# jinli99/iShapEditing

Measured on AMD Instinct MI355X. Metric: end-to-end drag-edit wall-clock (s) per shape, lower is better.
Workload: dtype f16; 1 GPU; C3 chair drag-edit: 3 handle->target pairs, 40 guided iterations (UNet fwd + drag gradient + UNet input-grad bwd + DDPM update) + 256^3 occupancy decode; unet=421M params, 1x96x128x128 latent, fp16 torso, r1=12, scale=1200

## Files before the change

include/ishap.h:

```cpp
#ifndef ISHAP_H
#define ISHAP_H
#ifdef __cplusplus
extern "C" {
#endif

const char* ishap_last_error(void);
int ishap_device_status(void);
int ishap_rendezvous_would_grant(const void* owner, void* stream);
int ishap_version(void);

typedef struct ishap_unet ishap_unet;

typedef struct {
  int image_size;
  int in_channels;
  int model_channels;
  int out_channels;
  int num_res_blocks;
  int n_mult;
  int channel_mult[8];
  int n_att;
  int attention_ds[8];
  int num_head_channels;
  int max_batch;
// ... 96 lines not shown
                        const float* grad_mul_dev, long long numel, float* out, void* stream);
int ishap_axpby(const float* x, const float* y, float a, float b, long long numel, float* out, void* stream);

typedef struct {
  int W;
  int ld;
  int Cc;
  const int* chmap;
  const float* sources;
  const float* targets;
  int B;
  int r;
  float voxel;
  float cof;
  int l1;
  unsigned char* touched;
  int* nmask;
  void* acc;
  void* grad_fx;
  unsigned char* chan_weight;
  const float* weights;
} ishap_drag_args;
int ishap_drag_setup(const ishap_drag_args* a, void* stream);
int ishap_drag_loss_grad(const ishap_drag_args* a, const void* edit_nhwc_f16, const void* orig_nhwc_f16,
                         float* grad_nhwc, float* loss, void* stream);
int ishap_drag_loss_cotangent(const ishap_drag_args* a, const void* edit_nhwc_f16, const void* orig_nhwc_f16,
                              float* grad_nhwc, float* loss, void* cot_f16, unsigned* bits, float* scale2, void* stream);
typedef struct {
  int E;
  int W, ld, Cc;
  const int* chmap;
  const float* sources;
  const float* targets;
  const int* handle_offsets;
  int r;
  float voxel;
  const float* cof;
  int l1;
  long long orig_stride;
  void* scratch;
  long long scratch_bytes;
  const float* weights;
  long long weights_stride;
} ishap_drag_batch_args;
long long ishap_drag_batch_scratch_bytes(int E, int W, int ld);
int ishap_drag_batch_setup(const ishap_drag_batch_args* a, void* stream);
// ... 244 lines not shown
```

ishapediting_amd/_lib.py:

```python
from __future__ import annotations

import ctypes as C
import os

HERE = os.path.dirname(os.path.abspath(__file__))
LIB_PATH = os.path.join(HERE, "libishap_hip.so")

c_float_p = C.POINTER(C.c_float)
c_void_p = C.c_void_p


class UNetConfigC(C.Structure):
    _fields_ = [("image_size", C.c_int), ("in_channels", C.c_int), ("model_channels", C.c_int),
                ("out_channels", C.c_int), ("num_res_blocks", C.c_int), ("n_mult", C.c_int),
                ("channel_mult", C.c_int * 8), ("n_att", C.c_int), ("attention_ds", C.c_int * 8),
                ("num_head_channels", C.c_int), ("max_batch", C.c_int)]


class StepCoefs(C.Structure):
    _fields_ = [("min_log", C.c_float), ("max_log", C.c_float), ("sqrt_recip", C.c_float),
                ("sqrt_recipm1", C.c_float), ("coef1", C.c_float), ("coef2", C.c_float),
                ("nonzero", C.c_float), ("clip_denoised", C.c_int), ("mode", C.c_int),
                ("ddim_a", C.c_float), ("ddim_b", C.c_float), ("ddim_sigma", C.c_float),
                ("rng", C.c_int), ("rng_seed", C.c_ulonglong), ("rng_offset", C.c_ulonglong), ("noise_out", c_void_p)]
# ... 92 lines not shown
    "ishap_unet_run_tail": (C.c_int, [c_void_p]),
    "ishap_unet_snapshot_save": (C.c_int, [c_void_p, c_void_p]),
    "ishap_unet_snapshot_restore": (C.c_int, [c_void_p, c_void_p]),
    "ishap_unet_snapshot_drop": (C.c_int, [c_void_p]),
    "ishap_unet_snapshot_bytes": (C.c_longlong, [c_void_p]),
    "ishap_unet_marks": (C.c_int, [c_void_p, c_void_p, c_void_p, C.c_int, c_void_p, c_void_p]),
    "ishap_unet_prepare_timesteps": (C.c_int, [c_void_p, c_void_p, C.c_int, c_void_p]),
    "ishap_unet_backward_input": (C.c_int, [c_void_p, c_void_p, c_void_p, c_void_p, c_void_p]),
    "ishap_unet_backward_from_output": (C.c_int, [c_void_p, c_void_p, C.c_int, c_void_p, c_void_p, c_void_p]),
    "ishap_triplane_points_loss_grad": (C.c_int, [c_void_p, C.c_int, C.POINTER(DecoderWeightsC), c_void_p, c_void_p, c_void_p,
                                                  c_void_p, C.c_longlong, c_void_p, c_void_p, c_void_p, c_void_p]),
    "ishap_x0_grad_to_cotangent": (C.c_int, [c_void_p, c_void_p, c_void_p, c_void_p, C.c_float, C.c_float, C.c_int, C.c_int,
                                             c_void_p, c_void_p, c_void_p]),
    "ishap_ddpm_step": (C.c_int, [c_void_p, c_void_p, c_void_p, c_void_p, C.POINTER(StepCoefs), C.c_int, C.c_int,
                                  C.c_int, c_void_p, c_void_p, c_void_p, c_void_p, c_void_p]),
    "ishap_ddpm_step_guided": (C.c_int, [c_void_p, c_void_p, c_void_p, c_void_p, C.POINTER(StepCoefs), C.c_int, C.c_int, C.c_int,
                                         c_void_p, C.c_float, c_void_p, c_void_p, c_void_p, c_void_p, c_void_p]),
    "ishap_ddpm_step_guided_scales": (C.c_int, [c_void_p, c_void_p, c_void_p, c_void_p, C.POINTER(StepCoefs), C.c_int, C.c_int,
                                                C.c_int, c_void_p, c_void_p, c_void_p, c_void_p, c_void_p, c_void_p, c_void_p]),
    "ishap_guided_update": (C.c_int, [c_void_p, c_void_p, c_void_p, C.c_float, c_void_p, C.c_longlong, c_void_p,
                                      c_void_p]),
    "ishap_axpby": (C.c_int, [c_void_p, c_void_p, C.c_float, C.c_float, C.c_longlong, c_void_p, c_void_p]),
    "ishap_drag_setup": (C.c_int, [C.POINTER(DragArgsC), c_void_p]),
    "ishap_drag_loss_grad": (C.c_int, [C.POINTER(DragArgsC), c_void_p, c_void_p, c_void_p, c_void_p, c_void_p]),
    "ishap_drag_loss_cotangent": (C.c_int, [C.POINTER(DragArgsC), c_void_p, c_void_p, c_void_p, c_void_p, c_void_p, c_void_p,
                                            c_void_p, c_void_p]),
    "ishap_drag_batch_scratch_bytes": (C.c_longlong, [C.c_int, C.c_int, C.c_int]),
    "ishap_drag_batch_setup": (C.c_int, [C.POINTER(DragBatchArgsC), c_void_p]),
    "ishap_drag_batch_loss_grad": (C.c_int, [C.POINTER(DragBatchArgsC), c_void_p, c_void_p, c_void_p, c_void_p, c_void_p]),
    "ishap_drag_batch_loss_cotangent": (C.c_int, [C.POINTER(DragBatchArgsC), c_void_p, c_void_p, c_void_p, c_void_p, c_void_p,
                                                  c_void_p, c_void_p, c_void_p]),
    "ishap_drag_track_scratch_bytes": (C.c_longlong, [C.c_int] * 5),
    "ishap_drag_track": (C.c_int, [c_void_p, c_void_p, C.c_longlong, C.c_int, C.c_int, C.c_int, c_void_p, c_void_p,
                                   C.POINTER(C.c_int), C.c_int, C.c_float, C.c_int, C.c_int, c_void_p, c_void_p, c_void_p, c_void_p,
                                   c_void_p, c_void_p, C.c_longlong, c_void_p]),
    "ishap_drag_retarget": (C.c_int, [C.POINTER(DragArgsC), c_void_p, c_void_p, C.c_float, C.c_float, c_void_p, c_void_p, c_void_p,
                                      c_void_p]),
    "ishap_drag_batch_retarget": (C.c_int, [C.POINTER(DragBatchArgsC), c_void_p, c_void_p, C.c_float, C.c_float, c_void_p, c_void_p,
                                            c_void_p, c_void_p]),
    "ishap_drag_batch_retarget_each": (C.c_int, [C.POINTER(DragBatchArgsC), c_void_p, c_void_p, C.POINTER(C.c_float),
                                                 C.POINTER(C.c_float), c_void_p, c_void_p, c_void_p, c_void_p]),
    "ishap_region_plane_weights_scratch_bytes": (C.c_longlong, [C.c_int]),
    "ishap_region_plane_weights": (C.c_int, [c_void_p, C.c_int, c_void_p, c_void_p, C.c_int, C.c_int, C.c_int, C.c_float, C.c_float,
                                             c_void_p, c_void_p, c_void_p, C.c_longlong, c_void_p]),
    "ishap_region_plane_marks": (C.c_int, [c_void_p, C.c_int, c_void_p, c_void_p, C.c_int, C.c_int, C.c_int, c_void_p, c_void_p,
                                           c_void_p, C.c_longlong, c_void_p]),
# ... 84 lines not shown
    "ishap_sparse_seed_range": (C.c_int, [C.c_int, C.c_int, C.c_int, C.POINTER(C.c_int), C.POINTER(C.c_int)]),
    "ishap_sparse_seed_volume": (C.c_int, [c_void_p, C.c_int, C.c_float, C.c_int, c_void_p, c_void_p]),
    "ishap_sparse_compact_scratch_bytes": (C.c_longlong, [C.c_int]),
    "ishap_sparse_compact": (C.c_int, [c_void_p, C.c_int, C.c_int, C.c_int, c_void_p, c_void_p, C.c_longlong, c_void_p, c_void_p,
                                       C.c_longlong, c_void_p]),
    "ishap_triplane_decode_bricks": (C.c_int, [c_void_p, C.c_int, C.POINTER(DecoderWeightsC), c_void_p, C.c_int, c_void_p,
                                               C.c_longlong, c_void_p, c_void_p]),
    "ishap_sparse_reach_bytes": (C.c_longlong, [C.c_longlong]),
    "ishap_sparse_grow": (C.c_int, [c_void_p, c_void_p, C.c_longlong, C.c_int, C.c_float, c_void_p, c_void_p, c_void_p, c_void_p,
                                    c_void_p]),
    "ishap_sparse_surface_scratch_bytes": (C.c_longlong, [C.c_int, C.c_longlong]),
    "ishap_sparse_surface_count": (C.c_int, [c_void_p, c_void_p, C.c_longlong, C.c_int, C.c_float, c_void_p, c_void_p, c_void_p,
                                             C.c_longlong, c_void_p, c_void_p]),
    "ishap_sparse_surface_emit": (C.c_int, [c_void_p, c_void_p, C.c_longlong, C.c_int, C.c_float, c_void_p, c_void_p, c_void_p,
                                            C.c_longlong, c_void_p, c_void_p, c_void_p]),
    "ishap_mesh_simplify_scratch_bytes": (C.c_longlong, [C.c_longlong, C.c_longlong, C.POINTER(C.c_int)]),
    "ishap_mesh_simplify_count": (C.c_int, [c_void_p, C.c_longlong, c_void_p, C.c_longlong, C.POINTER(C.c_double), C.c_double,
                                            C.POINTER(C.c_int), C.c_int, c_void_p, C.c_longlong, c_void_p, c_void_p]),
    "ishap_mesh_simplify_emit": (C.c_int, [c_void_p, C.c_longlong, c_void_p, C.c_longlong, C.POINTER(C.c_double), C.c_double,
                                           C.POINTER(C.c_int), C.c_int, C.c_double, c_void_p, C.c_longlong, c_void_p, c_void_p, c_void_p,
                                           c_void_p, c_void_p]),
}

ABI = 26

_lib = None


def lib():
    global _lib
    if _lib is None:
        if not os.path.exists(LIB_PATH):
            raise RuntimeError(
                f"{LIB_PATH} is missing: the HIP extension is required (no CPU fallback exists). "
                "Build it with `python -m ishapediting_amd.build`.")
        import torch
        tlib = os.path.join(os.path.dirname(torch.__file__), "lib", "libamdhip64.so")
        if os.path.exists(tlib):
            C.CDLL(tlib, mode=C.RTLD_GLOBAL)
        l = C.CDLL(LIB_PATH)
        for name, (res, args) in SYMBOLS.items():
            fn = getattr(l, name)
            fn.restype = res
            fn.argtypes = args
        if l.ishap_version() < ABI:
            raise RuntimeError(f"{LIB_PATH} is an older build (ABI {l.ishap_version()} < {ABI}): rebuild with `python -m ishapediting_amd.build`")
        _lib = l
# ... 60 lines not shown
```

ishapediting_amd/csrc/api.hip:

```cpp
#include "../../include/ishap.h"
#include "common.h"
#include "ddpm.h"
#include "decode.h"
#include "constrain.h"
#include "drag.h"
#include "track.h"
#include "retarget.h"
#include "regions.h"
#include "render.h"

static thread_local std::string g_err;
void ishap_set_error(const std::string& msg) { g_err = msg; }

#include <atomic>
#include <cmath>
#include <cstdio>
#include <cstring>
#include <mutex>
static std::atomic<unsigned*> g_status{nullptr};
static std::mutex g_status_mu;
unsigned* ishap_status_word() {
  unsigned* p = g_status.load(std::memory_order_acquire);
  if (p) return p;
  std::lock_guard<std::mutex> lk(g_status_mu);
// ... 214 lines not shown
}

static int fill_drag(const ishap_drag_args* a, DragBatchArgs& d) {
  ISHAP_REQUIRE(a && a->chmap && a->sources && a->targets && a->touched && a->nmask && a->acc && a->grad_fx && a->chan_weight,
                "null argument");
  ISHAP_REQUIRE(a->W > 1 && a->B >= 1 && a->r >= 0 && a->Cc >= 1 && a->ld >= 1, "drag dims");
  DragArgs& b = d.base;
  fill_drag_shared(a, b);
  b.touched = a->touched; b.nmask = a->nmask; b.acc = (long long*)a->acc; b.gfx = (long long*)a->grad_fx;
  b.chw = a->chan_weight;
  d.E = 1;
  d.orig_stride = 0;
  d.hoff[0] = 0; d.hoff[1] = a->B;
  d.cof[0] = a->cof;
  return 0;
}

int ishap_drag_setup(const ishap_drag_args* a, void* stream) {
  DragBatchArgs d;
  ISHAP_TRY(fill_drag(a, d));
  return drag_batch_setup_launch(d, (hipStream_t)stream);
}

int ishap_drag_loss_grad(const ishap_drag_args* a, const void* edit, const void* orig, float* grad, float* loss,
                         void* stream) {
  DragBatchArgs d;
  ISHAP_TRY(fill_drag(a, d));
  ISHAP_REQUIRE(edit && orig && grad && loss, "null argument");
  fill_drag_call(d, edit, orig, grad, loss);
  return drag_batch_loss_launch(d, nullptr, nullptr, nullptr, a->weights, 0, (hipStream_t)stream);
}

int ishap_drag_loss_cotangent(const ishap_drag_args* a, const void* edit, const void* orig, float* grad, float* loss,
                              void* cot_f16, unsigned* bits, float* scale2, void* stream) {
  DragBatchArgs d;
  ISHAP_TRY(fill_drag(a, d));
  ISHAP_REQUIRE(edit && orig && grad && loss && cot_f16 && bits && scale2, "null argument");
  fill_drag_call(d, edit, orig, grad, loss);
  return drag_batch_loss_launch(d, (half_t*)cot_f16, bits, scale2, a->weights, 0, (hipStream_t)stream);
}

struct DragBatchScratch { long long *gfx, *acc; int* nmask; unsigned char *touched, *chw; long long bytes; };
static DragBatchScratch drag_batch_carve(void* base, int E, int W, int ld) {
  Carve c{(char*)base};
  return {c.take<long long>((long long)E * W * W * ld), c.take<long long>(2ll * E), c.take<int>(E),
          c.take<unsigned char>(3ll * E * W * W), c.take<unsigned char>(3ll * ld), c.total()};
// ... 347 lines not shown
```

ishapediting_amd/csrc/drag.h:

```cpp
#pragma once
#include "common.h"
#include <algorithm>

__device__ __forceinline__ void plane_axes(int p, int& a_col, int& a_row) {
  a_col = (p == 1) ? 1 : 0;
  a_row = (p == 0) ? 1 : 2;
}

__device__ __forceinline__ float lattice(float s, float voxel, int k) {
#pragma clang fp contract(off)
  const float o = voxel * (float)k;
  return s + o;
}

struct Bilin { int x0, y0; float w[4]; };
__device__ __forceinline__ Bilin bilin_setup(float u, float v, int W) {
#pragma clang fp contract(off)
  Bilin b;
  const double ix = (((double)u + 1.0) / 2.0) * (double)(W - 1);
  const double iy = (((double)v + 1.0) / 2.0) * (double)(W - 1);
  const double fx = floor(ix), fy = floor(iy);
  b.x0 = (int)fx; b.y0 = (int)fy;
  const double wx1 = ix - fx, wx0 = 1.0 - wx1, wy1 = iy - fy, wy0 = 1.0 - wy1;
  b.w[0] = (float)(wx0 * wy0); b.w[1] = (float)(wx1 * wy0); b.w[2] = (float)(wx0 * wy1); b.w[3] = (float)(wx1 * wy1);
// ... 53 lines not shown
  int tblk[DRAG_MAX_EDITS + 1] = {};
  float cof[DRAG_MAX_EDITS] = {};
};
__device__ __forceinline__ DragArgs drag_edit_args(const DragBatchArgs& b, int e) {
  DragArgs a = b.base;
  const long long n = (long long)a.W * a.W * a.ld;
  const int h0 = b.hoff[e];
  a.edit += e * n;
  a.orig += e * b.orig_stride;
  a.sources += 3 * h0;
  a.targets += 3 * h0;
  a.B = b.hoff[e + 1] - h0;
  a.cof = b.cof[e];
  a.touched += (long long)e * 3 * a.W * a.W;
  a.nmask += e;
  a.grad += e * n;
  a.gfx += e * n;
  a.acc += 2 * e;
  a.loss += e;
  return a;
}
int drag_batch_check(const DragBatchArgs& a);
int drag_batch_setup_launch(DragBatchArgs& a, hipStream_t s);
int drag_batch_loss_launch(DragBatchArgs& a, half_t* cot, unsigned* bits, float* scale2, const float* weights, long long wstride,
                           hipStream_t s);
```

ishapediting_amd/csrc/drag.hip:

```cpp
#include "drag.h"
#include <cstdlib>


__device__ __forceinline__ void fx_add(long long* dst, float v, float scale) {
  atomicAdd(reinterpret_cast<unsigned long long*>(dst), (unsigned long long)__float2ll_rn(v * scale));
}
__device__ __forceinline__ void block_loss_add(float lsum, long long* dst) {
  __shared__ double red[4];
  double v = (double)lsum;
  for (int o = 32; o > 0; o >>= 1) v += __shfl_xor(v, o);
  if ((threadIdx.x & 63) == 0) red[threadIdx.x >> 6] = v;
  __syncthreads();
  if (threadIdx.x == 0)
    atomicAdd(reinterpret_cast<unsigned long long*>(dst),
              (unsigned long long)__double2ll_rn(((red[0] + red[1]) + (red[2] + red[3])) * (double)DRAG_ACC_SCALE));
}

constexpr int DSEG = 5;
__device__ __forceinline__ void drag_motion_body(const DragArgs& a, int blk, int nblk) {
  const int side = 2 * a.r + 1;
  const int nchunk = (a.Cc + 63) / 64;
  const int nseg = (side + DSEG - 1) / DSEG;
  const int nrows = 3 * a.B * side * nchunk * nseg;
  const int lane = threadIdx.x & 63;
// ... 77 lines not shown
      a00 += bt.w[0] * g; a01 += bt.w[1] * g; a10 += bt.w[2] * g; a11 += bt.w[3] * g;
    }
    if (open) { flush_col(xcur, a00, a10); flush_col(xcur + 1, a01, a11); }
  }
  block_loss_add(lsum, a.acc + 0);
}

__device__ __forceinline__ void drag_touch_one(const DragArgs& a, int p, int b, int st, int i, int j) {
  drag_touch_marks(a, p, b, st, i, j, [&](long long o, unsigned bit) {
    atomicOr(reinterpret_cast<unsigned*>(a.touched + (o & ~3ll)), bit << (8 * (o & 3)));
  });
}

__device__ __forceinline__ void drag_count_body(const DragArgs& a) {
  __shared__ int red[256];
  int cnt = 0;
  for (int i = threadIdx.x; i < 3 * a.W * a.W; i += 256) cnt += (a.touched[i] & 1) ? 0 : 1;
  red[threadIdx.x] = cnt;
  __syncthreads();
  for (int o = 128; o > 0; o >>= 1) { if (threadIdx.x < o) red[threadIdx.x] += red[threadIdx.x + o]; __syncthreads(); }
  if (threadIdx.x == 0) a.nmask[0] = red[0];
}

__global__ void drag_chan_weight_kernel(DragArgs a) {
  const int idx = blockIdx.x * blockDim.x + threadIdx.x;
  if (idx >= 3 * a.ld) return;
  const int p = idx / a.ld, ch = idx - p * a.ld;
  int cnt = 0;
  for (int c = 0; c < a.Cc; ++c) cnt += a.chmap[p * a.Cc + c] == ch ? 1 : 0;
  a.chw[idx] = (unsigned char)min(cnt, 255);
}

__device__ __forceinline__ void drag_finish(const DragArgs& a) {
  const int side = 2 * a.r + 1;
  const double ntot = 3.0 * (double)a.Cc * (double)a.B * (double)side * (double)side * (double)side;
  double loss = -((double)a.acc[0] * (1.0 / (double)DRAG_ACC_SCALE)) / ntot;
  if (a.cof > 0.f)
    loss -= (double)a.cof * ((double)a.acc[1] * (1.0 / (double)DRAG_ACC_SCALE)) / ((double)a.Cc * (double)a.nmask[0]);
  a.loss[0] = (float)loss;
  a.acc[0] = 0;
  a.acc[1] = 0;
}

template <bool WEIGHTED>
__device__ __forceinline__ void drag_gather_body(const DragArgs& a, int blk, int nblk, unsigned* __restrict__ absmax_bits,
                                                 const float* __restrict__ wmap) {
  typedef long long ll2 __attribute__((ext_vector_type(2)));
  typedef unsigned char uc8 __attribute__((ext_vector_type(8)));
  const long long n = (long long)a.W * a.W * a.ld;
  const int WW = a.W * a.W;
  const bool mask = a.cof > 0.f;
  const float denom = (float)a.Cc * (float)a.nmask[0];
  float m = 0.f, lsum = 0.f;
// ... 154 lines not shown
  ISHAP_REQUIRE((3 * a.base.W * a.base.W) % 4 == 0 && a.base.ld % 8 == 0,
                "drag: 3*W*W must be a multiple of 4 and the tap channels of 8");
  ISHAP_REQUIRE(a.hoff[0] == 0, "drag batch: handle_offsets[0] must be 0");
  for (int e = 0; e < a.E; ++e) ISHAP_REQUIRE(a.hoff[e + 1] > a.hoff[e], "drag batch: every edit needs at least one handle");
  return 0;
}

int drag_batch_setup_launch(DragBatchArgs& a, hipStream_t s) {
  ISHAP_TRY(drag_batch_check(a));
  const DragArgs& d = a.base;
  const int side = 2 * d.r + 1;
  const long long n = (long long)d.W * d.W * d.ld;
  ISHAP_CHECK_HIP(hipMemsetAsync(d.touched, 0, (size_t)a.E * 3 * d.W * d.W, s));
  ISHAP_CHECK_HIP(hipMemsetAsync(d.gfx, 0, (size_t)a.E * n * sizeof(long long), s));
  ISHAP_CHECK_HIP(hipMemsetAsync(d.acc, 0, (size_t)a.E * 2 * sizeof(long long), s));
  const int total = 3 * 2 * side * side * a.hoff[a.E];
  hipLaunchKernelGGL(drag_batch_touch_kernel, dim3(ceil_div(total, 256)), dim3(256), 0, s, a);
  hipLaunchKernelGGL(drag_batch_count_kernel, dim3(a.E), dim3(256), 0, s, a);
  hipLaunchKernelGGL(drag_chan_weight_kernel, dim3(ceil_div(3 * d.ld, 256)), dim3(256), 0, s, d);
  ISHAP_CHECK_HIP(hipGetLastError());
  return 0;
}

static unsigned gather_blocks(long long n) {
  constexpr int cap = 512;
  return (unsigned)std::min<long long>((n / 8 + 255) / 256, cap);
}

int drag_batch_loss_launch(DragBatchArgs& a, half_t* cot, unsigned* bits, float* scale2, const float* weights, long long wstride,
                           hipStream_t s) {
  ISHAP_TRY(drag_batch_check(a));
  ISHAP_REQUIRE(!weights || a.E == 1 || wstride == 0 || wstride >= 3ll * a.base.W * a.base.W,
                "drag: weights_stride must be 0 (one map for all edits) or at least 3*W*W");
  if (!cot) bits = nullptr;
  constexpr int cap = 1024;
  const int side = 2 * a.base.r + 1;
  a.tblk[0] = 0;
  for (int e = 0; e < a.E; ++e) {
    const int nrows = 3 * (a.hoff[e + 1] - a.hoff[e]) * side * ((a.base.Cc + 63) / 64) * ((side + DSEG - 1) / DSEG);
    a.tblk[e + 1] = a.tblk[e] + min(ceil_div(nrows * 64, 256), cap);
  }
  hipLaunchKernelGGL(drag_batch_terms_kernel, dim3(a.tblk[a.E]), dim3(256), 0, s, a, bits);
  const long long n = (long long)a.base.W * a.base.W * a.base.ld;
  const unsigned gb = gather_blocks(n);
  if (weights)
    hipLaunchKernelGGL(drag_batch_gather_weighted_kernel, dim3(gb * a.E), dim3(256), 0, s, a, (int)gb, bits, weights, wstride);
// ... 13 lines not shown
```

ishapediting_amd/csrc/unet.h:

```cpp
#pragma once
#include <functional>
#include <map>
#include <string>
#include <vector>

#include "../../include/ishap.h"
#include "common.h"

struct Tensor {
  half_t* p = nullptr;
  int N = 0, H = 0, W = 0, C = 0;
  long long* sums = nullptr;
  const half_t* cat_a = nullptr; const half_t* cat_b = nullptr; const long long* cat_sa = nullptr; const long long* cat_sb = nullptr;
  int cat_ca = 0;
  SlabSrc pend, cat_pend;
  long long rows() const { return (long long)N * H * W; }
  long long numel() const { return rows() * C; }
};

struct Arena {
  char* base = nullptr;
  size_t cap = 0, off = 0, high = 0;
  bool dry = false;
  void reset() { off = 0; }
// ... 102 lines not shown
  KeptForward kept;
  size_t bytes() const { return arena_cap + stat_cap * sizeof(long long) + film_cap * sizeof(float); }
};

struct ishap_unet {
  ishap_unet_config cfg;
  int device = 0;
  int ted = 0;
  int in_pad = 0;
  ConvW stem, head;
  NormW head_norm;
  std::vector<ResL> res;
  std::vector<AttnL> attn;
  std::vector<BlockL> in_blocks, out_blocks;
  BlockL mid;
  int final_ch = 0;
  float *te_w0 = nullptr, *te_b0 = nullptr, *te_w2 = nullptr, *te_b2 = nullptr;
  float *emb_w = nullptr, *emb_b = nullptr;
  int film_rows = 0;
  float *d_temb = nullptr, *d_e1 = nullptr, *d_emb = nullptr, *d_film = nullptr;
  float* film_cache = nullptr;
  size_t film_cache_rows = 0;
  std::vector<float> film_cache_ts;
  float *pc_temb = nullptr, *pc_e1 = nullptr, *pc_emb = nullptr;
  std::vector<ParamSlot> params;
  std::map<std::string, int> param_index;
  int n_loaded = 0;
  Arena arena;
  float* ws = nullptr;          size_t ws_floats = 0;
  float* gn_partial = nullptr;  size_t gn_partial_floats = 0;
  KeptForward kept;
  long long* stat_base = nullptr;
  size_t stat_cap = 0, stat_off = 0, stat_high = 0;
  unsigned long long seq = 0, grad_seq = 0;
  int grad_F = -1;
  hipStream_t side = nullptr;
  hipEvent_t ev_fork = nullptr, ev_tail = nullptr, ev_mid = nullptr;
  bool marks_on = false;
  std::vector<hipEvent_t> marks;
  std::vector<int> mark_tags;
  int marks_n = 0;
  hipEvent_t mark_tail_begin = nullptr, mark_tail_end = nullptr;
  bool mark_tail_set = false;
  bool tail_pending = false;
  std::vector<std::function<int(hipStream_t)>> tail_tape;
  bool tail_deferred = false, mid_recorded = false;
// ... 48 lines not shown
```

ishapediting_amd/csrc/unet.hip:

```cpp
#include "unet.h"

#include <cstring>

#include "attention.h"
#include "decode.h"
#include "misc.h"
#include "norm.h"

static int round_up(int a, int b) { return (a + b - 1) / b * b; }

static void init_conv(ConvW& c, const std::string& path, int cin, int cout, int taps) {
  c.path = path; c.cin = cin; c.cout = cout; c.taps = taps;
  c.kpad = round_up(cin, 32);
  c.cout_pad = round_up(cout, 32);
}

int unet_build(ishap_unet* u) {
  const ishap_unet_config& cfg = u->cfg;
  const int mc = cfg.model_channels;
  u->ted = mc * 4;
  u->in_pad = cfg.in_channels >= 64 ? round_up(cfg.in_channels, 64) : round_up(cfg.in_channels, 32);
  auto has_att = [&](int ds) {
    for (int i = 0; i < cfg.n_att; ++i) if (cfg.attention_ds[i] == ds) return true;
    return false;
// ... 609 lines not shown
  k.N = N;
  k.feat = feat_layer;
  k.tail_planned = overlap;
  k.have_saved = (keep & 1) != 0 && !dry;
  k.fwd_mark = u->arena.off;
  k.stat_fwd_mark = u->stat_off;
  k.bwd_since_fwd = 0;
  return 0;
}

template <typename T>
static int snap_reserve(T** buf, size_t* cap, size_t need) {
  if (need <= *cap) return 0;
  if (*buf) ISHAP_CHECK_HIP(hipFree(*buf));
  *buf = nullptr;
  *cap = 0;
  ISHAP_CHECK_HIP(hipMalloc((void**)buf, need * sizeof(T)));
  *cap = need;
  return 0;
}

extern "C" {

int ishap_version(void) { return 26; }

int ishap_unet_create(const ishap_unet_config* cfg, int device, ishap_unet** out) {
  ISHAP_REQUIRE(cfg && out, "null argument");
  ISHAP_REQUIRE(cfg->n_mult >= 1 && cfg->n_mult <= 8 && cfg->n_att <= 8, "config arrays");
  ISHAP_REQUIRE(cfg->model_channels % 32 == 0, "model_channels must be a multiple of 32 (GroupNorm32)");
  ISHAP_REQUIRE(cfg->num_head_channels > 0 && cfg->num_head_channels % 32 == 0, "num_head_channels % 32");
  ISHAP_REQUIRE(cfg->out_channels % 4 == 0, "out_channels % 4");
  ISHAP_REQUIRE(cfg->max_batch >= 1 && cfg->max_batch <= 16, "max_batch in [1,16]");
  int minres = cfg->image_size >> (cfg->n_mult - 1);
  ISHAP_REQUIRE(minres * minres >= 64 && (cfg->image_size & (cfg->image_size - 1)) == 0,
                "image_size: power of two with at least 8x8 at the deepest level");
  ISHAP_CHECK_HIP(hipSetDevice(device));
  ishap_unet* u = new ishap_unet();
  u->cfg = *cfg;
  u->marks_on = ishap_switch("ISHAP_BWD_MARKS", 0) != 0;
  u->device = device;
  int r = unet_build(u);
  if (r) { delete u; return r; }
  u->arena.dry = true;
  std::vector<float> ts(cfg->max_batch, 0.f);
  for (int nb = 1; nb <= cfg->max_batch && !r; ++nb) {
    r = unet_forward_impl(u, nullptr, ts.data(), nb, (int)u->out_blocks.size() - 1, nullptr, nullptr, 1, 0, true);
    if (!r) r = unet_backward_impl(u, nullptr, (const void*)0x1000, 0, nullptr, nullptr, 0, true);
// ... 51 lines not shown
  if (ndim) *ndim = p.ndim;
  if (shape) for (int i = 0; i < 4; ++i) shape[i] = p.shape[i];
  return 0;
}

int ishap_unet_load_param(ishap_unet* u, const char* name, const float* data, long long numel, void* stream) {
  ISHAP_REQUIRE(u && name && data, "null argument");
  auto it = u->param_index.find(name);
  ISHAP_REQUIRE(it != u->param_index.end(), std::string("unexpected key in state_dict: ") + name);
  ParamSlot& p = u->params[it->second];
  ISHAP_REQUIRE(p.numel() == numel, std::string("size mismatch for ") + name);
  ISHAP_CHECK_HIP(hipSetDevice(u->device));
  ISHAP_TRY(load_param(u, p, data, (hipStream_t)stream));
  if (!p.loaded) { p.loaded = true; u->n_loaded++; }
  u->film_cache_ts.clear();
  u->snap.valid = false;
  return 0;
}

int ishap_unet_prepare_timesteps(ishap_unet* u, const float* ts, int n, void* stream) {
  ISHAP_REQUIRE(u && (ts || n == 0) && n >= 0 && n <= 4096, "prepare_timesteps arguments");
  ISHAP_CHECK_HIP(hipSetDevice(u->device));
  hipStream_t s = (hipStream_t)stream;
  u->film_cache_ts.clear();
  if (u->kept.film != u->d_film) { u->kept.have_saved = false; u->kept.film = u->d_film; u->kept.film_ld = u->film_rows; }
  if (n == 0) return 0;
  ISHAP_REQUIRE(u->n_loaded == (int)u->params.size(), "prepare_timesteps before all parameters are loaded");
  const int mc = u->cfg.model_channels;
  if ((size_t)n > u->film_cache_rows) {
    if (u->film_cache) ISHAP_CHECK_HIP(hipFree(u->film_cache));
    u->film_cache = nullptr;
    u->film_cache_rows = 0;
    ISHAP_CHECK_HIP(hipMalloc((void**)&u->film_cache, (size_t)n * u->film_rows * sizeof(float)));
    u->film_cache_rows = (size_t)n;
  }
  if (!u->pc_temb) {
    ISHAP_CHECK_HIP(hipMalloc((void**)&u->pc_temb, (size_t)16 * mc * sizeof(float)));
    ISHAP_CHECK_HIP(hipMalloc((void**)&u->pc_e1, (size_t)16 * u->ted * sizeof(float)));
    ISHAP_CHECK_HIP(hipMalloc((void**)&u->pc_emb, (size_t)16 * u->ted * sizeof(float)));
  }
  for (int c0 = 0; c0 < n; c0 += 16) {
    const int m = std::min(16, n - c0);
    TsArg ta;
    for (int i = 0; i < 16; ++i) ta.t[i] = i < m ? ts[c0 + i] : 0.f;
    ISHAP_TRY(timestep_embedding(ta, u->pc_temb, m, mc, s));
    ISHAP_TRY(gemv_f32(u->te_w0, u->te_b0, u->pc_temb, u->pc_e1, u->ted, mc, m, 0, s));
    ISHAP_TRY(gemv_f32(u->te_w2, u->te_b2, u->pc_e1, u->pc_emb, u->ted, u->ted, m, 1, s));
    ISHAP_TRY(gemv_f32(u->emb_w, u->emb_b, u->pc_emb, u->film_cache + (size_t)c0 * u->film_rows, u->film_rows, u->ted, m, 1, s));
  }
  u->film_cache_ts.assign(ts, ts + n);
  return 0;
}

int ishap_unet_params_loaded(const ishap_unet* u) { return u ? u->n_loaded : 0; }

int ishap_unet_join_tail(ishap_unet* u, void* stream) {
  ISHAP_REQUIRE(u, "null argument");
  ISHAP_CHECK_HIP(hipSetDevice(u->device));
  return unet_join_tail(u, (hipStream_t)stream);
}

int ishap_unet_run_tail(ishap_unet* u) {
  ISHAP_REQUIRE(u, "null argument");
  ISHAP_CHECK_HIP(hipSetDevice(u->device));
  return unet_run_tail(u);
}

int ishap_unet_forward(ishap_unet* u, const float* x, const float* timesteps, int N, int feat_layer, float* out,
                       void* inter_feat, int keep_for_backward, void* stream) {
  ISHAP_REQUIRE(u && x && timesteps && out, "null argument");
  ISHAP_REQUIRE(u->n_loaded == (int)u->params.size(), "missing keys: not every state_dict tensor has been loaded");
  ISHAP_TRY(ishap_check_status());
  ISHAP_CHECK_HIP(hipSetDevice(u->device));
// ... 142 lines not shown
```

ishapediting_amd/drag_utils.py:

```python
from __future__ import annotations

import argparse
import collections
import copy
import ctypes as C
import os
from argparse import Namespace
from typing import List, Optional

import numpy as np
import torch as th

from . import _lib
from .script_util import args_to_dict, create_model_and_diffusion, model_and_diffusion_defaults
from .triplane_decoder import MultiTriplane, decode_planes_grid, decode_volume, prepare_planes
from . import mesh as mesh_backend
from .volume import clean_volume


def get_args(argv=None):
    parser = argparse.ArgumentParser(description="Generate a set of triplane and their corresponding meshes")
    parser.add_argument("--resolution", type=str, default=128, required=False)
    parser.add_argument("--num_steps", type=int, default=200, required=False)
    parser.add_argument("--shape_resolution", type=int, default=256, required=False)
# ... 32 lines not shown
    e = half - half % 3
    idx = _nearest_channel_index(half, e) if half % 3 else np.arange(half)
    per = e // 3
    out = np.zeros((3, 2 * per), dtype=np.int32)
    for p in range(3):
        out[p, :per] = idx[p * per:(p + 1) * per]
        out[p, per:] = half + idx[p * per:(p + 1) * per]
    return out


def resize_feat_align(feature, cat_var=True):
    batch_num, channel_num = feature.shape[:2]
    assert not channel_num % 2 and batch_num == 1
    cm = th.as_tensor(feat_channel_map(channel_num), device=feature.device, dtype=th.long)
    per = cm.shape[1] // 2
    if not cat_var:
        cm = cm[:, :per]
    return feature[0][cm.reshape(-1)].reshape(3, -1, feature.shape[2], feature.shape[3]).type(th.float32)


_FUSED_UPDATE = os.environ.get("ISHAP_FUSED_UPDATE", "1") == "1"
_OVERLAP_TAIL = os.environ.get("ISHAP_OVERLAP_TAIL", "1") == "1"
_FIRST_STEP_REUSE = os.environ.get("ISHAP_FIRST_STEP_REUSE", "1") == "1"


class _DragKernelsBase:

    def __init__(self, device, W: int, ld: int, chmap, r: int, voxel: float, loss_type: str):
        self.device = th.device(device)
        self.W, self.ld, self.r, self.voxel = W, ld, r, float(voxel)
        self.l1 = 1 if loss_type == "l1" else 0
        self.chmap = th.as_tensor(np.asarray(chmap), dtype=th.int32).reshape(3, -1).contiguous().to(self.device)
        self.Cc = self.chmap.shape[1]
        self.bits = th.zeros(1, dtype=th.int32, device=self.device)
        self.scale2 = th.ones(2, dtype=th.float32, device=self.device)
        self.sources = self.targets = None
        self._L = _lib.lib()
        self.goals = self.remaining = self.arrived = self.done = None
        self._aim_ptr = None
        self._aim_keep = None

    def _call(self, name: str, *args):
        _lib.call(self.device, name, *args)

    def _targets_ptr(self) -> int:
        return self.targets.data_ptr() if self._aim_ptr is None else self._aim_ptr
# ... 10 lines not shown
        if tuple(K.shape) != (H, 3):
            raise ValueError(f"retarget: K must be [{H}, 3], got {tuple(K.shape)}")
        if self.goals is None:
            self.goals = th.empty((H, 3), dtype=th.float32, device=self.device)
            self.remaining = th.empty(H, dtype=th.float32, device=self.device)
            self.arrived = th.empty(H, dtype=th.int32, device=self.device)
            self.done = th.empty(E, dtype=th.int32, device=self.device)
        self.retarget_raw(K.data_ptr(), self.goals.data_ptr(), self.remaining.data_ptr(), self.arrived.data_ptr(),
                          self.done.data_ptr(), step, arrive)
        return self.goals, self.remaining, self.arrived, self.done

    def retarget_raw(self, k: int, goals: int, remaining: int, arrived: int, done: int, step, arrive):
        keep, self._aim_ptr = self._aim_ptr, goals
        try:
            self._retarget_call(k, remaining, arrived, done, step, arrive)
        except Exception:
            self._aim_ptr = keep
            raise

    def _weight_map(self, w):
        return check_weight_map(w, self.W).to(device=self.device).contiguous()


def check_weight_map(w, W: int) -> th.Tensor:
    w = w.detach() if th.is_tensor(w) else th.as_tensor(np.asarray(w))
    if tuple(w.shape) != (3, W, W):
        raise ValueError(f"weights must be a [3, {W}, {W}] map (one [row, col] slice per plane), got {tuple(w.shape)}")
    w = w.to(th.float32)
    if not bool(th.isfinite(w).all()) or bool((w < 0).any()):
        raise ValueError("weights must be finite and >= 0")
    return w


def check_region_cof(cof: float, has_regions: bool, what: str = "cof"):
    if has_regions and not cof > 0:
        raise ValueError(f"{what} = {cof}: keep / free regions and weights scale the preservation term, which needs cof > 0")


class DragKernels(_DragKernelsBase):

    def __init__(self, device, W: int, ld: int, chmap, r: int, voxel: float, loss_type: str = "l2"):
        super().__init__(device, W, ld, chmap, r, voxel, loss_type)
        self.touched = th.zeros(3 * W * W, dtype=th.uint8, device=self.device)
        self.nmask = th.zeros(1, dtype=th.int32, device=self.device)
        self.chan_weight = th.zeros(3 * ld, dtype=th.uint8, device=self.device)
        self.acc = th.zeros(2, dtype=th.int64, device=self.device)
        self.gfx = th.zeros(W * W * ld, dtype=th.int64, device=self.device)
        self.grad = th.empty((W * W, ld), dtype=th.float32, device=self.device)
        self.loss = th.zeros(1, dtype=th.float32, device=self.device)
        self.cot = th.empty((W * W, ld), dtype=th.float16, device=self.device)
        self.cof = 0.0
        self.weights = None

    def _args(self) -> _lib.DragArgsC:
        return _lib.DragArgsC(self.W, self.ld, self.Cc, self.chmap.data_ptr(), self.sources.data_ptr(),
                              self._targets_ptr(), self.sources.shape[0], self.r, self.voxel, float(self.cof),
                              self.l1, self.touched.data_ptr(), self.nmask.data_ptr(), self.acc.data_ptr(), self.gfx.data_ptr(),
                              self.chan_weight.data_ptr(), _lib.ptr(self.weights))

    def setup(self, sources, targets, cof: float, weights=None):
        check_region_cof(float(cof), weights is not None)
        self.weights = None if weights is None else self._weight_map(weights)

        def pts(v):
            v = v.detach() if th.is_tensor(v) else th.as_tensor(np.asarray(v))
            return v.to(device=self.device, dtype=th.float32).reshape(-1, 3).contiguous()
        self.sources, self.targets = pts(sources), pts(targets)
        assert self.sources.shape[0] == self.targets.shape[0]
        self.cof = float(cof)
        self._reset_aim()
        self._call("ishap_drag_setup", C.byref(self._args()))

    def _retarget_call(self, k, remaining, arrived, done, step, arrive):
        self._call("ishap_drag_retarget", C.byref(self._args()), self.targets.data_ptr(), k, float(step), float(arrive),
                   remaining, arrived, done)

    def loss_grad_ptr(self, edit_ptr: int, orig_ptr: int):
        self._call("ishap_drag_loss_grad", C.byref(self._args()), edit_ptr, orig_ptr, self.grad.data_ptr(),
                   self.loss.data_ptr())
        return self.grad, self.loss

    def loss_grad(self, edit: th.Tensor, orig: th.Tensor):
        assert edit.dtype == th.float16 and orig.dtype == th.float16 and edit.is_contiguous() and orig.is_contiguous()
        return self.loss_grad_ptr(edit.data_ptr(), orig.data_ptr())

    def loss_cotangent_ptr(self, edit_ptr: int, orig_ptr: int, orig_stride: int = 0, loss_out=None):
        assert orig_stride == 0
        loss = self.loss if loss_out is None else loss_out
        self._call("ishap_drag_loss_cotangent", C.byref(self._args()), edit_ptr, orig_ptr, self.grad.data_ptr(),
                   loss.data_ptr(), self.cot.data_ptr(), self.bits.data_ptr(), self.scale2.data_ptr())
        return self.cot, self.scale2

    def scaled_cotangent(self):
        self._call("ishap_grad_to_scaled_f16", self.grad.data_ptr(), self.cot.data_ptr(), self.bits.data_ptr(),
# ... 450 lines not shown
    means, stds = (np.asarray(v, dtype=np.float32).reshape(-1) for v in (means, stds))
    if means.size != 96 or stds.size != 96:
        raise ValueError(f"triplane statistics must hold 96 values each, not {means.size} and {stds.size}")
    return means, stds


class DragStuff:

    args = get_args()
    overlap_tail = None
    _w = None
    _shape_gen = 0
    _first_step = None

    @property
    def w(self):
        return self._w

    @w.setter
    def w(self, value):
        self._w = value
        self._shape_changed()

    def _shape_changed(self):
        self._shape_gen = self._shape_gen + 1
        self._first_step = None

    def _first_step_key(self, overlap):
        w = self._w
        return (self._shape_gen, id(self.model), id(w), getattr(w, "_version", None), tuple(w.shape), self.args.feat_layer,
                self.args.w_time, tuple(getattr(self.diffusion, "timestep_map", ())), bool(overlap))

    def __init__(self, device=None, args=None, max_edits=1):
        if args is not None:
            self.args = args
        if int(max_edits) < 1:
            raise ValueError(f"max_edits must be >= 1, not {max_edits}")
        self.max_edits = int(max_edits)
        self.device = th.device("cuda", th.cuda.current_device()) if device is None else th.device(device)
        self.model, self.diffusion = create_model_and_diffusion(
            **args_to_dict(self.args, model_and_diffusion_defaults().keys()), device=self.device, max_batch=self.max_edits)
        self.model.eval()
        self.decoder = MultiTriplane(1, input_dim=3, output_dim=1, device=self.device)
        self.decoder.eval()
        self.range = 1.
        self.middle = 0.
        self.latent_code = None
        self.w0 = None
        self.w = None
        self.r1 = 12
        self.offset1 = make_offsets(self.r1, self.device)
        self.voxel_size = 2. / self.args.shape_resolution
        self.train_flag = True
        self.targets = None
        self.sources = None
        self.mesh = None
        self.mesh0 = None
        self.tri_feat0 = None
        self.last_volume_losses: List[th.Tensor] = []
        self.volume = None
        self.clean = None
        self.refine = None
        self.mesh_resolution = None
        self.mesh_simplify = None
        self.noise = []
        self.variance = []
        self.variance_noise = []
        self.feature_guidance: List[th.Tensor] = []
        self.last_losses: List[float] = []
        self.last_track = None
        self.last_stop = None
        self._dk: Optional[DragKernels] = None
        self.step_noise = None
        self.w_batch = None
        self.w0_batch = None
        self.feature_guidance_batch: List[th.Tensor] = []
        self.meshes0 = []
        self.meshes = []
# ... 222 lines not shown
        return _ClosedLoop(dk, trk, copts)

    def _loop_track(self, topts, width, ch, sources):
        if topts is None:
            return None
        tracker = HandleTracker(self.device, W=width, ld=ch, chmap=feat_channel_map(ch), voxel=self.voxel_size,
                                radius=topts["radius"], patch=topts["patch"])
        return _LoopTrack(tracker, sources, self.args.w_time, topts["every"])

    def handle_error(self):
        if self.last_track is None:
            raise RuntimeError("handle_error: no tracked edit has run (training(..., track=True))")
        tracks = self.last_track if isinstance(self.last_track, list) else [self.last_track]
        out = []
        for tr, (src, tgt) in zip(tracks, self._track_ends):
            if len(tr["steps"]) == 0:
                raise RuntimeError("handle_error: the tracked edit stopped before its first tracked step")
            pos, move = tr["positions"][-1], tgt - src
            m2 = (move * move).sum(-1)
            frac = th.where(m2 > 0, ((pos - src) * move).sum(-1) / m2.clamp_min(1e-30), th.ones_like(m2))
            out.append({"error": (pos - tgt).norm(dim=-1) / self.voxel_size, "fraction": frac})
        return out if isinstance(self.last_track, list) else out[0]

    def training(self, sources=None, targets=None, scale=600, cof=0.2, keep=None, free=None, keep_weight=4.0, free_weight=0.0,
                 region_dilate=0, weights=None, track=None, closed_loop=None, region_falloff=0.0, volume_keep=None, carve=None,
                 fill=None, volume_scale=None, volume_points=16384, volume_res=128):
        copts = closed_loop_options(closed_loop)
        topts = track_options(closed_loop_track(copts, track))
        if self.args.num_samples > 1:
            raise NotImplementedError("We can handle only one shape at each time!")
        ch, width = self.model.tap_shape(self.args.feat_layer)
        wmap = self._region_weights(width, cof, keep, free, keep_weight, free_weight, region_dilate, weights, region_falloff=region_falloff)
        cons, ratio = self._volume_constraints(scale, volume_keep, carve, fill, volume_scale, volume_points, volume_res)
        self.sources = th.tensor(np.asarray(sources), device=self.device, dtype=th.float32)
        self.targets = th.tensor(np.asarray(targets), device=self.device, dtype=th.float32)
        assert self.sources.shape[0] == self.targets.shape[0]
        img = self.w.clone().detach()
        dk = DragKernels(self.device, W=width, ld=ch, chmap=feat_channel_map(ch), r=self.r1, voxel=self.voxel_size,
                         loss_type=self.args.loss_type)
        dk.setup(self.sources, self.targets, cof, **({} if wmap is None else {"weights": wmap}))
        self._dk = dk
        trk = self._loop_track(topts, width, ch, [self.sources])
        cl = None if copts is None else self._closed_loop(dk, trk, copts)
        vol = None if cons is None else VolumeGuidance(self, cons, ratio)
        img, stop_time = yield from self._guided_loop(img, dk, self.feature_guidance, 0, [float(scale)], float(scale), vol is None,
                                                      **({} if trk is None else {"trk": trk}), **({} if cl is None else {"cl": cl}),
                                                      **({} if vol is None else {"vol": vol}))
        if trk is not None:
            res = trk.results() if cl is None else cl.results(trk.results())
            self.last_track, self._track_ends = res[0], [(self.sources, self.targets)]
        self.mesh = self.get_mesh(img=img, t=stop_time)

    def training_part(self, part, rigid, handles=16, start=None, scale=600, cof=0.2, keep=None, keep_weight=4.0, free_weight=0.0,
                      region_dilate=0, track=None, closed_loop=None, margin=0.0, region_falloff=0.0, solid=False, volume_scale=None,
                      volume_points=16384):
        from . import regions
        self.part_plan = plan = regions.plan_part_edit(part, rigid, handles=handles, start=start, **({} if margin == 0 else {"margin": margin}))
        self.part_solid = None
        vkw = {}
        if solid:
            left = part.mask.to(plan.moved.mask.device) & ~plan.moved.mask
            self.part_solid = {"fill": plan.moved, "carve": regions.Voxels(left) if bool(left.any()) else None}
            vkw = dict(fill=plan.moved, carve=self.part_solid["carve"], volume_scale=volume_scale, volume_points=volume_points,
                       volume_res=part.D)
        return self.training(plan.sources, plan.targets, scale=scale, cof=cof, keep=keep, free=plan.free, keep_weight=keep_weight,
                             free_weight=free_weight, region_dilate=region_dilate, region_falloff=region_falloff,
                             **({} if track is None else {"track": track}),
                             **({} if closed_loop is None else {"closed_loop": closed_loop}), **vkw)

    def _check_edits(self, K: int):
        check_edit_count(K, self.max_edits)

    def update_latent_params_batch(self, imgs, **kwargs):
# ... 227 lines not shown
```

Before: 0.1620 s/shape.

## Fuse drag setup into one edit kernel and cache per-edit host state

```diff
diff --git a/include/ishap.h b/include/ishap.h
--- a/include/ishap.h
+++ b/include/ishap.h
@@ -142,6 +142,7 @@
   const float* weights;
 } ishap_drag_args;
 int ishap_drag_setup(const ishap_drag_args* a, void* stream);
+int ishap_drag_setup_edit(const ishap_drag_args* a, const float* sources, const float* targets, void* stream);
 int ishap_drag_loss_grad(const ishap_drag_args* a, const void* edit_nhwc_f16, const void* orig_nhwc_f16,
                          float* grad_nhwc, float* loss, void* stream);
 int ishap_drag_loss_cotangent(const ishap_drag_args* a, const void* edit_nhwc_f16, const void* orig_nhwc_f16,
diff --git a/ishapediting_amd/_lib.py b/ishapediting_amd/_lib.py
--- a/ishapediting_amd/_lib.py
+++ b/ishapediting_amd/_lib.py
@@ -138,6 +138,7 @@
                                       c_void_p]),
     "ishap_axpby": (C.c_int, [c_void_p, c_void_p, C.c_float, C.c_float, C.c_longlong, c_void_p, c_void_p]),
     "ishap_drag_setup": (C.c_int, [C.POINTER(DragArgsC), c_void_p]),
+    "ishap_drag_setup_edit": (C.c_int, [C.POINTER(DragArgsC), c_void_p, c_void_p, c_void_p]),
     "ishap_drag_loss_grad": (C.c_int, [C.POINTER(DragArgsC), c_void_p, c_void_p, c_void_p, c_void_p, c_void_p]),
     "ishap_drag_loss_cotangent": (C.c_int, [C.POINTER(DragArgsC), c_void_p, c_void_p, c_void_p, c_void_p, c_void_p, c_void_p,
                                             c_void_p, c_void_p]),
@@ -268,7 +269,7 @@
                                            c_void_p, c_void_p]),
 }
 
-ABI = 26
+ABI = 27
 
 _lib = None
 
diff --git a/ishapediting_amd/csrc/api.hip b/ishapediting_amd/csrc/api.hip
--- a/ishapediting_amd/csrc/api.hip
+++ b/ishapediting_amd/csrc/api.hip
@@ -260,6 +260,13 @@
   return drag_batch_setup_launch(d, (hipStream_t)stream);
 }
 
+int ishap_drag_setup_edit(const ishap_drag_args* a, const float* sources, const float* targets, void* stream) {
+  ISHAP_REQUIRE(a && a->B >= 1 && a->B <= DRAG_SETUP_MAX_HANDLES, "drag setup_edit: 1..64 handles");
+  DragBatchArgs d;
+  ISHAP_TRY(fill_drag(a, d));
+  return drag_setup_edit_launch(d, sources, targets, (hipStream_t)stream);
+}
+
 int ishap_drag_loss_grad(const ishap_drag_args* a, const void* edit, const void* orig, float* grad, float* loss,
                          void* stream) {
   DragBatchArgs d;
diff --git a/ishapediting_amd/csrc/drag.h b/ishapediting_amd/csrc/drag.h
--- a/ishapediting_amd/csrc/drag.h
+++ b/ishapediting_amd/csrc/drag.h
@@ -99,5 +99,10 @@
 }
 int drag_batch_check(const DragBatchArgs& a);
 int drag_batch_setup_launch(DragBatchArgs& a, hipStream_t s);
+constexpr int DRAG_SETUP_MAX_HANDLES = 64;
+constexpr int DRAG_SETUP_THREADS = 1024;
+constexpr int DRAG_SETUP_SLICE = 4096;
+struct DragEditHandles { float src[3 * DRAG_SETUP_MAX_HANDLES], tgt[3 * DRAG_SETUP_MAX_HANDLES]; };
+int drag_setup_edit_launch(DragBatchArgs& a, const float* src, const float* tgt, hipStream_t s);
 int drag_batch_loss_launch(DragBatchArgs& a, half_t* cot, unsigned* bits, float* scale2, const float* weights, long long wstride,
                            hipStream_t s);
diff --git a/ishapediting_amd/csrc/drag.hip b/ishapediting_amd/csrc/drag.hip
--- a/ishapediting_amd/csrc/drag.hip
+++ b/ishapediting_amd/csrc/drag.hip
@@ -123,13 +123,16 @@
   if (threadIdx.x == 0) a.nmask[0] = red[0];
 }
 
-__global__ void drag_chan_weight_kernel(DragArgs a) {
-  const int idx = blockIdx.x * blockDim.x + threadIdx.x;
-  if (idx >= 3 * a.ld) return;
+__device__ __forceinline__ void drag_chan_weight_one(const DragArgs& a, int idx) {
   const int p = idx / a.ld, ch = idx - p * a.ld;
   int cnt = 0;
   for (int c = 0; c < a.Cc; ++c) cnt += a.chmap[p * a.Cc + c] == ch ? 1 : 0;
   a.chw[idx] = (unsigned char)min(cnt, 255);
+}
+__global__ void drag_chan_weight_kernel(DragArgs a) {
+  const int idx = blockIdx.x * blockDim.x + threadIdx.x;
+  if (idx >= 3 * a.ld) return;
+  drag_chan_weight_one(a, idx);
 }
 
 __device__ __forceinline__ void drag_finish(const DragArgs& a) {
@@ -330,6 +333,101 @@
   return 0;
 }
 
+__global__ __launch_bounds__(DRAG_SETUP_THREADS) void drag_setup_edit_kernel(DragArgs a, DragEditHandles h) {
+  typedef unsigned u32x4 __attribute__((ext_vector_type(4)));
+  __shared__ __attribute__((aligned(16))) unsigned char slice[DRAG_SETUP_SLICE];
+  __shared__ float pts[2][3 * DRAG_SETUP_MAX_HANDLES];
+  __shared__ int red[DRAG_SETUP_THREADS / 64];
+  const int tid = threadIdx.x, g = blockIdx.x, G = gridDim.x;
+  const int nbytes = 3 * a.W * a.W;
+  const int lo = g * DRAG_SETUP_SLICE, hi = min(lo + DRAG_SETUP_SLICE, nbytes);
+  float* const src_out = const_cast<float*>(a.sources);
+  float* const tgt_out = const_cast<float*>(a.targets);
+  for (int i = tid; i < 3 * a.B; i += DRAG_SETUP_THREADS) {
+    const float s = h.src[i], t = h.tgt[i];
+    pts[0][i] = s; pts[1][i] = t;
+    if (g == 0) { src_out[i] = s; tgt_out[i] = t; }
+  }
+  unsigned* words = reinterpret_cast<unsigned*>(slice);
+  for (int i = tid; i < DRAG_SETUP_SLICE / 4; i += DRAG_SETUP_THREADS) words[i] = 0u;
+  for (int idx = g * DRAG_SETUP_THREADS + tid; idx < 3 * a.ld; idx += G * DRAG_SETUP_THREADS) drag_chan_weight_one(a, idx);
+  __syncthreads();
+
+  DragArgs m = a;
+  m.sources = pts[0];
+  m.targets = pts[1];
+  const int side = 2 * a.r + 1, per = 2 * side * side * a.B;
+  const int WW = a.W * a.W;
+  for (int p = lo / WW; p <= (hi - 1) / WW; ++p)
+    for (int idx = tid; idx < per; idx += DRAG_SETUP_THREADS) {
+      int rem = idx;
+      const int j = rem % side; rem /= side;
+      const int i = rem % side; rem /= side;
+      const int st = rem % 2;
+      const int b = rem / 2;
+      drag_touch_marks(m, p, b, st, i, j, [&](long long o, unsigned bit) {
+        if (o < lo || o >= hi) return;
+        unsigned* w = words + (((int)o - lo) >> 2);
+        const unsigned mk = bit << (8 * (int)(o & 3));
+        if ((__atomic_load_n(w, __ATOMIC_RELAXED) & mk) != mk) atomicOr(w, mk);
+      });
+    }
+  __syncthreads();
+
+  const int nwords = (hi - lo) >> 2;
+  unsigned char* out = a.touched + lo;
+  const bool vec = ((hi - lo) & 15) == 0 && (reinterpret_cast<unsigned long long>(out) & 15ull) == 0;
+  const int nvec = vec ? nwords >> 2 : 0;
+  int untouched = 0;
+  auto clear0 = [](unsigned w) { return 4 - __popc(w & 0x01010101u); };
+  for (int i = tid; i < nvec; i += DRAG_SETUP_THREADS) {
+    const u32x4 v = reinterpret_cast<const u32x4*>(slice)[i];
+    reinterpret_cast<u32x4*>(out)[i] = v;
+    untouched += (clear0(v[0]) + clear0(v[1])) + (clear0(v[2]) + clear0(v[3]));
+  }
+  for (int i = 4 * nvec + tid; i < nwords; i += DRAG_SETUP_THREADS) {
+    const unsigned w = words[i];
+    reinterpret_cast<unsigned*>(out)[i] = w;
+    untouched += clear0(w);
+  }
+  for (int o = 32; o > 0; o >>= 1) untouched += __shfl_xor(untouched, o);
+  if ((tid & 63) == 0) red[tid >> 6] = untouched;
+  __syncthreads();
+  if (tid == 0) {
+    int u = 0;
+#pragma unroll
+    for (int k = 0; k < DRAG_SETUP_THREADS / 64; ++k) u += red[k];
+    const unsigned long long mine = (1ull << 32) | (unsigned long long)u;
+    const unsigned long long seen = atomicAdd(reinterpret_cast<unsigned long long*>(a.acc), mine);
+    if ((seen >> 32) == (unsigned long long)(G - 1)) {
+      a.nmask[0] = (int)(unsigned)(seen & 0xffffffffull) + u;
+      a.acc[0] = 0;
+      a.acc[1] = 0;
+    }
+  }
+}
+
+int drag_setup_edit_launch(DragBatchArgs& a, const float* src, const float* tgt, hipStream_t s) {
+  ISHAP_REQUIRE(src && tgt, "drag setup_edit: null argument");
+  ISHAP_REQUIRE(a.E == 1, "drag setup_edit: one edit");
+  const DragArgs& d = a.base;
+  const int B = a.hoff[1];
+  ISHAP_REQUIRE(B >= 1 && B <= DRAG_SETUP_MAX_HANDLES, "drag setup_edit: 1..64 handles");
+  ISHAP_TRY(drag_batch_check(a));
+  const long long side = 2ll * d.r + 1;
+  ISHAP_REQUIRE(d.W <= 16384 && 2 * side * side * B < (1ll << 31) - DRAG_SETUP_THREADS, "drag setup_edit: too many lattice points or texels");
+  ISHAP_REQUIRE((reinterpret_cast<unsigned long long>(d.touched) & 3ull) == 0 && (reinterpret_cast<unsigned long long>(d.acc) & 7ull) == 0,
+                "drag setup_edit: touched must be 4-byte and acc 8-byte aligned");
+  DragEditHandles h;
+  for (int i = 0; i < 3 * DRAG_SETUP_MAX_HANDLES; ++i) { h.src[i] = i < 3 * B ? src[i] : 0.f; h.tgt[i] = i < 3 * B ? tgt[i] : 0.f; }
+  DragArgs one = d;
+  one.B = B;
+  one.cof = a.cof[0];
+  hipLaunchKernelGGL(drag_setup_edit_kernel, dim3(ceil_div(3 * d.W * d.W, DRAG_SETUP_SLICE)), dim3(DRAG_SETUP_THREADS), 0, s, one, h);
+  ISHAP_CHECK_HIP(hipGetLastError());
+  return 0;
+}
+
 static unsigned gather_blocks(long long n) {
   constexpr int cap = 512;
   return (unsigned)std::min<long long>((n / 8 + 255) / 256, cap);
diff --git a/ishapediting_amd/csrc/unet.h b/ishapediting_amd/csrc/unet.h
--- a/ishapediting_amd/csrc/unet.h
+++ b/ishapediting_amd/csrc/unet.h
@@ -148,6 +148,7 @@
   float* film_cache = nullptr;
   size_t film_cache_rows = 0;
   std::vector<float> film_cache_ts;
+  hipStream_t film_cache_stream = nullptr;
   float *pc_temb = nullptr, *pc_e1 = nullptr, *pc_emb = nullptr;
   std::vector<ParamSlot> params;
   std::map<std::string, int> param_index;
diff --git a/ishapediting_amd/csrc/unet.hip b/ishapediting_amd/csrc/unet.hip
--- a/ishapediting_amd/csrc/unet.hip
+++ b/ishapediting_amd/csrc/unet.hip
@@ -1,5 +1,6 @@
 #include "unet.h"
 
+#include <algorithm>
 #include <cstring>
 
 #include "attention.h"
@@ -655,7 +656,7 @@
 
 extern "C" {
 
-int ishap_version(void) { return 26; }
+int ishap_version(void) { return 27; }
 
 int ishap_unet_create(const ishap_unet_config* cfg, int device, ishap_unet** out) {
   ISHAP_REQUIRE(cfg && out, "null argument");
@@ -753,6 +754,8 @@
   ISHAP_REQUIRE(u && (ts || n == 0) && n >= 0 && n <= 4096, "prepare_timesteps arguments");
   ISHAP_CHECK_HIP(hipSetDevice(u->device));
   hipStream_t s = (hipStream_t)stream;
+  if (n > 0 && (size_t)n == u->film_cache_ts.size() && s == u->film_cache_stream && std::equal(ts, ts + n, u->film_cache_ts.begin()))
+    return 0;
   u->film_cache_ts.clear();
   if (u->kept.film != u->d_film) { u->kept.have_saved = false; u->kept.film = u->d_film; u->kept.film_ld = u->film_rows; }
   if (n == 0) return 0;
@@ -780,6 +783,7 @@
     ISHAP_TRY(gemv_f32(u->emb_w, u->emb_b, u->pc_emb, u->film_cache + (size_t)c0 * u->film_rows, u->film_rows, u->ted, m, 1, s));
   }
   u->film_cache_ts.assign(ts, ts + n);
+  u->film_cache_stream = s;
   return 0;
 }
 
diff --git a/ishapediting_amd/drag_utils.py b/ishapediting_amd/drag_utils.py
--- a/ishapediting_amd/drag_utils.py
+++ b/ishapediting_amd/drag_utils.py
@@ -78,6 +78,7 @@
 _FUSED_UPDATE = os.environ.get("ISHAP_FUSED_UPDATE", "1") == "1"
 _OVERLAP_TAIL = os.environ.get("ISHAP_OVERLAP_TAIL", "1") == "1"
 _FIRST_STEP_REUSE = os.environ.get("ISHAP_FIRST_STEP_REUSE", "1") == "1"
+_EDIT_SETUP = os.environ.get("ISHAP_EDIT_SETUP", "1") == "1"
 
 
 class _DragKernelsBase:
@@ -134,6 +135,10 @@
         return check_weight_map(w, self.W).to(device=self.device).contiguous()
 
 
+def _handle_count(v) -> int:
+    return max(int(np.prod(np.shape(v))) // 3, 0)
+
+
 def check_weight_map(w, W: int) -> th.Tensor:
     w = w.detach() if th.is_tensor(w) else th.as_tensor(np.asarray(w))
     if tuple(w.shape) != (3, W, W):
@@ -164,14 +169,19 @@
         self.cof = 0.0
         self.weights = None
 
-    def _args(self) -> _lib.DragArgsC:
-        return _lib.DragArgsC(self.W, self.ld, self.Cc, self.chmap.data_ptr(), self.sources.data_ptr(),
-                              self._targets_ptr(), self.sources.shape[0], self.r, self.voxel, float(self.cof),
+    MAX_EDIT_HANDLES = 64
+
+    def _args(self, handles=None) -> _lib.DragArgsC:
+        src, tgt, B = handles or (self.sources.data_ptr(), self._targets_ptr(), self.sources.shape[0])
+        return _lib.DragArgsC(self.W, self.ld, self.Cc, self.chmap.data_ptr(), src, tgt, B, self.r, self.voxel, float(self.cof),
                               self.l1, self.touched.data_ptr(), self.nmask.data_ptr(), self.acc.data_ptr(), self.gfx.data_ptr(),
                               self.chan_weight.data_ptr(), _lib.ptr(self.weights))
 
     def setup(self, sources, targets, cof: float, weights=None):
         check_region_cof(float(cof), weights is not None)
+        on_host = not any(th.is_tensor(v) and v.is_cuda for v in (sources, targets))
+        if _EDIT_SETUP and weights is None and on_host and 1 <= _handle_count(sources) <= self.MAX_EDIT_HANDLES:
+            return self.setup_edit(sources, targets, cof)
         self.weights = None if weights is None else self._weight_map(weights)
 
         def pts(v):
@@ -182,6 +192,24 @@
         self.cof = float(cof)
         self._reset_aim()
         self._call("ishap_drag_setup", C.byref(self._args()))
+
+    def setup_edit(self, sources, targets, cof: float):
+        host = lambda v: np.ascontiguousarray(np.asarray(v.detach().cpu() if th.is_tensor(v) else v, dtype=np.float32).reshape(-1, 3))
+        src, tgt = host(sources), host(targets)
+        if src.shape != tgt.shape:
+            raise ValueError(f"setup_edit: {src.shape[0]} sources and {tgt.shape[0]} targets (need the same count)")
+        n = src.shape[0]
+        pair = th.empty((2, n, 3), dtype=th.float32, device=self.device)
+        keep = self.cof, self.weights
+        self.cof, self.weights = float(cof), None
+        try:
+            self._call("ishap_drag_setup_edit", C.byref(self._args((pair[0].data_ptr() if n else None, pair[1].data_ptr() if n else None, n))),
+                       src.ctypes.data, tgt.ctypes.data)
+        except Exception:
+            self.cof, self.weights = keep
+            raise
+        self.sources, self.targets = pair[0], pair[1]
+        self._reset_aim()
 
     def _retarget_call(self, k, remaining, arrived, done, step, arrive):
         self._call("ishap_drag_retarget", C.byref(self._args()), self.targets.data_ptr(), k, float(step), float(arrive),
@@ -678,6 +706,16 @@
         self._w = value
         self._shape_changed()
 
+    @property
+    def sources(self):
+        dk = getattr(self, "_dk", None)
+        return None if dk is None else dk.sources
+
+    @property
+    def targets(self):
+        dk = getattr(self, "_dk", None)
+        return None if dk is None else dk.targets
+
     def _shape_changed(self):
         self._shape_gen = self._shape_gen + 1
         self._first_step = None
@@ -708,8 +746,6 @@
         self.offset1 = make_offsets(self.r1, self.device)
         self.voxel_size = 2. / self.args.shape_resolution
         self.train_flag = True
-        self.targets = None
-        self.sources = None
         self.mesh = None
         self.mesh0 = None
         self.tri_feat0 = None
@@ -978,6 +1014,15 @@
             out.append({"error": (pos - tgt).norm(dim=-1) / self.voxel_size, "fraction": frac})
         return out if isinstance(self.last_track, list) else out[0]
 
+    def _plain_kernels(self, width, ch):
+        key = (int(width), int(ch), int(self.r1), float(self.voxel_size), self.args.loss_type, str(self.device))
+        kept = getattr(self, "_dk_plain", None)
+        if kept is None or kept[0] != key:
+            kept = (key, DragKernels(self.device, W=width, ld=ch, chmap=feat_channel_map(ch), r=self.r1, voxel=self.voxel_size,
+                                     loss_type=self.args.loss_type))
+            self._dk_plain = kept
+        return kept[1]
+
     def training(self, sources=None, targets=None, scale=600, cof=0.2, keep=None, free=None, keep_weight=4.0, free_weight=0.0,
                  region_dilate=0, weights=None, track=None, closed_loop=None, region_falloff=0.0, volume_keep=None, carve=None,
                  fill=None, volume_scale=None, volume_points=16384, volume_res=128):
@@ -988,15 +1033,18 @@
         ch, width = self.model.tap_shape(self.args.feat_layer)
         wmap = self._region_weights(width, cof, keep, free, keep_weight, free_weight, region_dilate, weights, region_falloff=region_falloff)
         cons, ratio = self._volume_constraints(scale, volume_keep, carve, fill, volume_scale, volume_points, volume_res)
-        self.sources = th.tensor(np.asarray(sources), device=self.device, dtype=th.float32)
-        self.targets = th.tensor(np.asarray(targets), device=self.device, dtype=th.float32)
-        assert self.sources.shape[0] == self.targets.shape[0]
-        img = self.w.clone().detach()
-        dk = DragKernels(self.device, W=width, ld=ch, chmap=feat_channel_map(ch), r=self.r1, voxel=self.voxel_size,
-                         loss_type=self.args.loss_type)
-        dk.setup(self.sources, self.targets, cof, **({} if wmap is None else {"weights": wmap}))
+        src = th.tensor(np.asarray(sources), dtype=th.float32)
+        tgt = th.tensor(np.asarray(targets), dtype=th.float32)
+        assert src.shape[0] == tgt.shape[0]
+        img = self.w.detach()
+        if _EDIT_SETUP and wmap is None and topts is None and copts is None:
+            dk = self._plain_kernels(width, ch)
+        else:
+            dk = DragKernels(self.device, W=width, ld=ch, chmap=feat_channel_map(ch), r=self.r1, voxel=self.voxel_size,
+                             loss_type=self.args.loss_type)
+        dk.setup(src, tgt, cof, **({} if wmap is None else {"weights": wmap}))
         self._dk = dk
-        trk = self._loop_track(topts, width, ch, [self.sources])
+        trk = None if topts is None else self._loop_track(topts, width, ch, [dk.sources])
         cl = None if copts is None else self._closed_loop(dk, trk, copts)
         vol = None if cons is None else VolumeGuidance(self, cons, ratio)
         img, stop_time = yield from self._guided_loop(img, dk, self.feature_guidance, 0, [float(scale)], float(scale), vol is None,
@@ -1004,7 +1052,7 @@
                                                       **({} if vol is None else {"vol": vol}))
         if trk is not None:
             res = trk.results() if cl is None else cl.results(trk.results())
-            self.last_track, self._track_ends = res[0], [(self.sources, self.targets)]
+            self.last_track, self._track_ends = res[0], [(dk.sources, dk.targets)]
         self.mesh = self.get_mesh(img=img, t=stop_time)
 
     def training_part(self, part, rigid, handles=16, start=None, scale=600, cof=0.2, keep=None, keep_weight=4.0, free_weight=0.0,
```

Result: no change. 0.1611 s/shape (median of 4 runs) (-0.6%).
